# josefmaierfl/matchinglib_poselib

Hardware: AMD Instinct MI355X
Metric: descriptor-pairs/s (8k x 8k ORB BF-Hamming kNN=2 + ratio) (higher is better)
Workload: dtype fp4 (E2M1 MFMA, f32 accumulate: exact); 1 GPU; C2: 8192x8192 ORB-256 BF-Hamming kNN=2 + 0.75 ratio + DMatch rows, 64 image pair(s) per GPU per step; pairs_per_gpu=64, settle_steps=400, solver_polish=1

## Files before the change

include/mlpl_debug.h:

```cpp
#ifndef MLPL_DEBUG_H
#define MLPL_DEBUG_H
#include "mlpl_c.h"

#ifdef __cplusplus
extern "C" {
#endif

int mlpl_debug_arrsac_trace(mlpl_ctx *ctx, int32_t *buf, int cap);

int mlpl_debug_usac_trace(mlpl_ctx *ctx, double *buf, int cap_records);

int mlpl_debug_ransac_draw(mlpl_ctx *ctx, long long out[2]);

long long mlpl_debug_fiber_selftest(int n, int workers, int rounds);

int mlpl_debug_eig9(mlpl_ctx *ctx, const double *G, const double *start, int count, double *out12, double *jacobi10);

int mlpl_debug_dk_stats(mlpl_ctx *ctx, int enable, int stats[16]);

int mlpl_debug_l2_flags(mlpl_ctx *ctx, int flags[4]);

int mlpl_debug_hamming_stamps(mlpl_ctx *ctx, unsigned long long *out, int max_items);

int mlpl_debug_hamming_clock(mlpl_ctx *ctx, unsigned long long *out, int max_items);

int mlpl_debug_hop_trace(mlpl_ctx *ctx, float *us, int *codes, int max_items, long long *ws_grows);

int mlpl_debug_last_kernels(mlpl_ctx *ctx, int out[13]);

int mlpl_debug_last_l2_match(mlpl_ctx *ctx, int out[4]);

int mlpl_debug_l2_fold_counts(mlpl_ctx *ctx, const float *d_q, int nq, size_t q_stride, size_t q_batch_stride, const float *d_t, int nt,
                              size_t t_stride, size_t t_batch_stride, int dim, int ratio_test, float ratio, int batch, int32_t *d_idx, float *d_dist,
                              int32_t *counts);

int mlpl_debug_count_pass(mlpl_ctx *ctx, const double *p1, const double *p2, int n, const double *E, int n_live, int n_bound,
                          const int32_t *ids, int table_len, double thresh2, int point_splits, int32_t *table_inout);

#ifdef __cplusplus
}
#endif
#endif
```

matchinglib_poselib_amd/_lib.py:

```python
from __future__ import annotations

import ctypes as C
import os
import threading

_HERE = os.path.dirname(os.path.abspath(__file__))
_LIB_PATH = os.environ.get("MLPL_LIB_PATH") or os.path.join(_HERE, "lib", "libmlpl_hip.so")

MLPL_OK = 0
MLPL_E_BAD_INPUT = -1
MLPL_E_UNSUPPORTED = -2
MLPL_E_FAILED = -3
MLPL_E_INTERNAL = -103
MLPL_E_FEW_KEYPOINTS = -4
MLPL_E_NO_DEVICE = -100
MLPL_E_HIP = -101
MLPL_E_NOMEM = -102


class MlplError(RuntimeError):
    def __init__(self, code: int, where: str, msg: str = ""):
        self.code = code
        super().__init__(f"{where} failed with code {code}: {msg}")

# ... 76 lines not shown
    "mlpl_usac_essential": (c_int, [c_void_p, c_void_p, c_void_p, c_int, c_void_p, c_void_p, c_void_p, c_void_p]),
    "mlpl_usac_essential_dev": (c_int, [c_void_p, c_void_p, c_void_p, c_int, c_void_p, c_void_p, c_void_p, c_void_p, c_void_p]),
    "mlpl_usac_essential_batch_dev": (c_int, [c_void_p, c_int, c_void_p, c_void_p, c_int, c_void_p, c_void_p, c_void_p, c_void_p, c_void_p, c_void_p,
                                              c_void_p, c_void_p, c_int, c_void_p, c_void_p]),
    "mlpl_usac_last_stats": (c_int, [c_void_p, c_void_p]),
    "mlpl_usac_last_degeneracy": (c_int, [c_void_p, c_void_p, c_void_p, c_void_p, c_int]),
    "mlpl_debug_usac_trace": (c_int, [c_void_p, c_void_p, c_int]),
    "mlpl_ransac_essential": (c_int, [c_void_p, c_void_p, c_void_p, c_int, c_double, c_double, c_int, c_int, c_u32,
                                      c_void_p, c_void_p, C.POINTER(c_int), C.POINTER(c_int)]),
    "mlpl_ransac_essential_dev": (c_int, [c_void_p, c_void_p, c_void_p, c_int, c_double, c_double, c_int, c_int,
                                          c_u32, c_void_p, c_void_p, C.POINTER(c_int), C.POINTER(c_int), c_void_p]),
    "mlpl_solve_5pt": (c_int, [c_void_p, c_void_p, c_void_p, c_int, c_void_p, c_int, c_void_p, c_void_p]),
    "mlpl_score_models": (c_int, [c_void_p, c_void_p, c_void_p, c_int, c_void_p, c_int, c_double, c_void_p,
                                  c_void_p]),
    "mlpl_ransac_last_stats": (c_int, [c_void_p, c_void_p]),
    "mlpl_debug_ransac_draw": (c_int, [c_void_p, c_void_p]),
    "mlpl_debug_fiber_selftest": (C.c_longlong, [c_int, c_int, c_int]),
    "mlpl_debug_eig9": (c_int, [c_void_p, c_void_p, c_void_p, c_int, c_void_p, c_void_p]),
    "mlpl_debug_dk_stats": (c_int, [c_void_p, c_int, c_void_p]),
    "mlpl_debug_hamming_stamps": (c_int, [c_void_p, c_void_p, c_int]),
    "mlpl_debug_hamming_clock": (c_int, [c_void_p, c_void_p, c_int]),
    "mlpl_debug_hop_trace": (c_int, [c_void_p, c_void_p, c_void_p, c_int, c_void_p]),
    "mlpl_debug_last_kernels": (c_int, [c_void_p, c_void_p]),
    "mlpl_debug_count_pass": (c_int, [c_void_p, c_void_p, c_void_p, c_int, c_void_p, c_int, c_int, c_void_p, c_int, c_double, c_int,
                                      c_void_p]),
    "mlpl_pair_pose_dev": (c_int, [c_void_p, c_void_p, c_int, c_void_p, c_int, c_int, c_void_p, c_void_p, c_void_p, c_void_p, c_double,
                                   c_int, c_double, c_int, c_u32, c_double, c_void_p, c_void_p]),
    "mlpl_pair_pose_batch_dev": (c_int, [c_void_p, c_int, c_void_p, c_int, c_void_p, c_int, c_int, c_void_p, c_void_p, c_void_p, c_void_p, c_double,
                                         c_int, c_double, c_int, c_void_p, c_double, c_void_p, c_void_p, c_void_p]),
    "mlpl_pair_pose_f32_dev": (c_int, [c_void_p, c_void_p, c_int, c_void_p, c_int, c_int, c_void_p, c_void_p, c_void_p, c_void_p, c_double,
                                       c_int, c_double, c_int, c_u32, c_double, c_void_p, c_void_p]),
    "mlpl_pair_pose_batch_f32_dev": (c_int, [c_void_p, c_int, c_void_p, c_int, c_void_p, c_int, c_int, c_void_p, c_void_p, c_void_p, c_void_p, c_double,
                                             c_int, c_double, c_int, c_void_p, c_double, c_void_p, c_void_p, c_void_p]),
    "mlpl_pair_pose_batch_usac_f32_dev": (c_int, [c_void_p, c_int, c_void_p, c_int, c_void_p, c_int, c_int, c_void_p, c_void_p, c_void_p, c_void_p, c_void_p, c_int,
                                                  c_void_p, c_double, c_void_p, c_void_p, c_void_p]),
    "mlpl_pair_pose_batch_arrsac_f32_dev": (c_int, [c_void_p, c_int, c_void_p, c_int, c_void_p, c_int, c_int, c_void_p, c_void_p, c_void_p, c_void_p, c_double, c_int,
                                                    c_void_p, c_double, c_void_p, c_void_p, c_void_p]),
    "mlpl_pair_pose_batch_lanes_dev": (c_int, [c_void_p, c_void_p, c_int, c_int, c_void_p, c_int, c_void_p, c_int, c_int, c_void_p, c_void_p, c_void_p, c_void_p,
                                               c_double, c_int, c_double, c_void_p, c_double, c_void_p, c_void_p, c_void_p]),
    "mlpl_pair_pose_batch_usac_dev": (c_int, [c_void_p, c_int, c_void_p, c_int, c_void_p, c_int, c_int, c_void_p, c_void_p, c_void_p, c_void_p, c_void_p, c_int,
                                              c_void_p, c_double, c_void_p, c_void_p, c_void_p]),
    "mlpl_pair_pose_batch_arrsac_dev": (c_int, [c_void_p, c_int, c_void_p, c_int, c_void_p, c_int, c_int, c_void_p, c_void_p, c_void_p, c_void_p, c_double, c_int,
                                                c_void_p, c_double, c_void_p, c_void_p, c_void_p]),
    "mlpl_sorted_match_idx": (c_int, [c_void_p, c_int, c_void_p]),
    "mlpl_pair_batch_last_stats": (c_int, [c_void_p, c_void_p]),
    "mlpl_ransac_essential_batch_dev": (c_int, [c_void_p, c_int, c_void_p, c_void_p, c_int, c_void_p, c_double, c_int, c_double, c_void_p, c_int, c_double,
# ... 112 lines not shown
        return self._lib

    def stream(self) -> int:
        return int(self._lib.mlpl_ctx_stream(self._h) or 0)

    def synchronize(self):
        check(self._lib.mlpl_ctx_synchronize(self._h), "mlpl_ctx_synchronize")

    def set_option(self, name: str, value: int):
        check(self._lib.mlpl_set_option(self._h, name.encode(), int(value)), "mlpl_set_option")

    def get_option(self, name: str) -> int:
        v = C.c_int(0)
        check(self._lib.mlpl_get_option(self._h, name.encode(), C.byref(v)), "mlpl_get_option")
        return v.value

    def last_kernels(self) -> list:
        out = (C.c_int * 13)()
        n = self._lib.mlpl_debug_last_kernels(self._h, out)
        if n < 0:
            raise MlplError(n, "mlpl_debug_last_kernels", last_error())
        return list(out[:n])

    def last_l2_match(self) -> list:
        out = (C.c_int * 4)()
        n = self._lib.mlpl_debug_last_l2_match(self._h, out)
        if n < 0:
            raise MlplError(n, "mlpl_debug_last_l2_match", last_error())
        return list(out[:n])

    def close(self):
        if getattr(self, "_h", None) is not None and self._h:
            self._lib.mlpl_ctx_destroy(self._h)
            self._h = None

    def __del__(self):
        try:
            self.close()
        except Exception:
            pass

    def __enter__(self):
        return self

    def __exit__(self, *exc):
        self.close()
# ... 15 lines not shown
```

matchinglib_poselib_amd/csrc/capi.hip:

```cpp

#include <algorithm>
#include <cfloat>
#include <cstdlib>
#include <cstring>
#include <new>

#include "mlpl_internal.h"

namespace mlpl {

static thread_local char g_err[512] = "";

void set_error(const char *fmt, ...) {
    va_list ap;
    va_start(ap, fmt);
    vsnprintf(g_err, sizeof(g_err), fmt, ap);
    va_end(ap);
}

int ws_get(mlpl_ctx *ctx, WsSlot slot, size_t bytes, void **out) {
    if (bytes < 4096) bytes = 4096;
    if (ctx->ws_bytes[slot] < bytes) {
        MLPL_HIP_TRY(hipDeviceSynchronize());
        if (ctx->ws[slot]) MLPL_HIP_TRY(hipFree(ctx->ws[slot]));
// ... 90 lines not shown
    MLPL_HIP_TRY(hipSetDevice(device_ordinal));
    hipDeviceProp_t prop;
    MLPL_HIP_TRY(hipGetDeviceProperties(&prop, device_ordinal));
    if (std::strncmp(prop.gcnArchName, "gfx950", 6) != 0) {
        set_error("device %d is %s; this library carries gfx950 code objects only", device_ordinal, prop.gcnArchName);
        return MLPL_E_NO_DEVICE;
    }
    mlpl_ctx *ctx = new (std::nothrow) mlpl_ctx();
    if (!ctx) return MLPL_E_NOMEM;
    std::memset(ctx, 0, sizeof(*ctx));
    ctx->device = device_ordinal;
    ctx->num_cus = prop.multiProcessorCount > 0 ? prop.multiProcessorCount : 256;
    ctx->opt_hamming_variant = 3;
    ctx->opt_hamming_qpl = 1;
    ctx->opt_hamming_blocks_per_cu = 32;
    ctx->opt_hamming_mfma_blocks_per_cu = 3;
    ctx->opt_hamming_mfma_qt = 0;
    ctx->opt_hamming_mfma_lds = 1;
    ctx->opt_hamming_mfma_weighted = 1;
    ctx->opt_hamming_mfma_prio = 0;
    ctx->opt_hamming_fused_merge = 1;
    ctx->opt_hamming_expand_fine = 1;
    ctx->opt_hamming_expand_inkernel = 1;
    ctx->opt_hamming_merge_emit = 0;
    ctx->opt_ransac_lazy_sums = 1;
    ctx->opt_ransac_overlap = 1;
    ctx->opt_ransac_f32_filter = 1;
    ctx->opt_ransac_count_mpl = 2;
    ctx->opt_ransac_count_tiles = 2;
    ctx->opt_ransac_count_wpe = 5;
    ctx->opt_ransac_count_threads = 256;
    ctx->opt_ransac_count_defer = 1;
    ctx->opt_pair_batch_feed = 1;
    ctx->opt_solver_polish = 1;
    ctx->opt_solver_wave3 = 1;
    ctx->opt_ransac_device_draw = 1;
    ctx->opt_usac_lo_warm_start = 1;
    ctx->opt_usac_lo5_fused_fit = 1;
    ctx->opt_hub_blocking_sync = 1;
    ctx->opt_eig_inverse_iteration = 1;
    ctx->opt_arrsac_refine_warm_start = 1;
    ctx->opt_usac_sprt_fast = 1;
    ctx->opt_l2_float_mfma = 1;
    ctx->opt_l2_fold_counts = 1;
    ctx->opt_vfc_store_u = 0;
    hipError_t e = hipStreamCreateWithFlags(&ctx->stream, hipStreamNonBlocking);
// ... 40 lines not shown
    if (ctx->stream) (void)hipStreamDestroy(ctx->stream);
    for (int i = 0; i < 2; ++i)
        if (ctx->aux_stream[i]) (void)hipStreamDestroy(ctx->aux_stream[i]);
    for (int i = 0; i < 8; ++i)
        if (ctx->aux_ev[i]) (void)hipEventDestroy(ctx->aux_ev[i]);
    delete ctx;
}

void *mlpl_ctx_stream(mlpl_ctx *ctx) { return ctx ? (void *)ctx->stream : nullptr; }
int mlpl_ctx_device(mlpl_ctx *ctx) { return ctx ? ctx->device : -1; }
int mlpl_ctx_synchronize(mlpl_ctx *ctx) {
    if (!ctx) return MLPL_E_BAD_INPUT;
    MLPL_HIP_TRY(hipStreamSynchronize(ctx->stream));
    return MLPL_OK;
}

static const struct {
    const char *name;
    int mlpl_ctx::*field;
    int lo, hi;
} kRangeOptions[] = {
    {"l2_fold_counts", &mlpl_ctx::opt_l2_fold_counts, 0, 1},
    {"hamming_expand_inkernel", &mlpl_ctx::opt_hamming_expand_inkernel, 0, 1},
    {"vfc_store_u", &mlpl_ctx::opt_vfc_store_u, 0, 1},
};

int mlpl_set_option(mlpl_ctx *ctx, const char *name, int value) {
    if (!ctx || !name) return MLPL_E_BAD_INPUT;
    for (const auto &o : kRangeOptions)
        if (!std::strcmp(name, o.name)) {
            if (value < o.lo || value > o.hi) {
                set_error("mlpl_set_option: unknown option or bad value: %s=%d", name, value);
                return MLPL_E_BAD_INPUT;
            }
            ctx->*(o.field) = value;
            return MLPL_OK;
        }
    if (!std::strcmp(name, "hamming_variant") && value >= 0 && value <= 3) ctx->opt_hamming_variant = value;
    else if (!std::strcmp(name, "hamming_mfma_qt") && (value == 0 || value == 1 || value == 2 || value == 4)) ctx->opt_hamming_mfma_qt = value;
    else if (!std::strcmp(name, "hamming_mfma_blocks_per_cu") && value >= 1 && value <= 64) ctx->opt_hamming_mfma_blocks_per_cu = value;
    else if (!std::strcmp(name, "hamming_mfma_lds") && (value >= 0 && value <= 2)) ctx->opt_hamming_mfma_lds = value;
    else if (!std::strcmp(name, "hamming_expand_fine") && (value == 0 || value == 1)) ctx->opt_hamming_expand_fine = value;
    else if (!std::strcmp(name, "hamming_mfma_prio") && (value == 0 || value == 1 || value == 3)) ctx->opt_hamming_mfma_prio = value;
    else if (!std::strcmp(name, "hamming_mfma_prefetch") && (value == 0 || value == 2 || value == 4 || value == 6)) ctx->opt_hamming_mfma_prefetch = value;
    else if (!std::strcmp(name, "hamming_split_rows") && (value == 0 || value == 4096 || value == 8192)) ctx->opt_hamming_split_rows = value;
    else if (!std::strcmp(name, "hamming_mfma_waves") && (value == 0 || value == 4 || value == 8 || value == 16)) ctx->opt_hamming_mfma_waves = value;
    else if (!std::strcmp(name, "hamming_mfma_weighted") && (value == 0 || value == 1)) ctx->opt_hamming_mfma_weighted = value;
    else if (!std::strcmp(name, "hamming_fused_merge") && (value == 0 || value == 1)) ctx->opt_hamming_fused_merge = value;
    else if (!std::strcmp(name, "hamming_stamps") && (value >= 0 && value <= 2)) ctx->opt_hamming_stamps = value;
    else if (!std::strcmp(name, "hamming_train01") && (value == 0 || value == 1)) ctx->opt_hamming_train01 = value;
    else if (!std::strcmp(name, "hamming_merge_emit") && (value == 0 || value == 1)) ctx->opt_hamming_merge_emit = value;
    else if (!std::strcmp(name, "l2_mfma_waves") && (value == 0 || value == 4 || value == 8)) ctx->opt_l2_mfma_waves = value;
    else if (!std::strcmp(name, "l2_mfma_blocks_per_cu") && value >= 0 && value <= 16) ctx->opt_l2_mfma_blocks_per_cu = value;
    else if (!std::strcmp(name, "hamming_qpl") && (value == 1 || value == 2)) ctx->opt_hamming_qpl = value;
// ... 90 lines not shown
    else if (!std::strcmp(name, "pair_batch_feed")) *value = ctx->opt_pair_batch_feed;
    else if (!std::strcmp(name, "pair_batch_raw_cap")) *value = ctx->opt_pair_batch_raw_cap;
    else if (!std::strcmp(name, "usac_lo_stepwise")) *value = ctx->opt_usac_lo_stepwise;
    else if (!std::strcmp(name, "usac_lo_warm_start")) *value = ctx->opt_usac_lo_warm_start;
    else if (!std::strcmp(name, "usac_first_batch")) *value = ctx->opt_usac_first_batch;
    else if (!std::strcmp(name, "usac_lo5_fused_fit")) *value = ctx->opt_usac_lo5_fused_fit;
    else if (!std::strcmp(name, "usac_sprt_fast")) *value = ctx->opt_usac_sprt_fast;
    else if (!std::strcmp(name, "ransac_host_table")) *value = ctx->opt_ransac_host_table;
    else if (!std::strcmp(name, "ransac_chunk")) *value = ctx->opt_ransac_chunk;
    else {
        set_error("mlpl_get_option: unknown option: %s", name);
        return MLPL_E_BAD_INPUT;
    }
    return MLPL_OK;
}

int mlpl_debug_last_kernels(mlpl_ctx *ctx, int out[13]) {
    if (!ctx || !out) return MLPL_E_BAD_INPUT;
    out[0] = ctx->dbg_count_kernel[0], out[1] = ctx->dbg_count_kernel[1];
    for (int i = 0; i < 11; ++i) out[2 + i] = ctx->dbg_hamming_kernel[i];
    return 13;
}

int mlpl_debug_last_l2_match(mlpl_ctx *ctx, int out[4]) {
    if (!ctx || !out) return MLPL_E_BAD_INPUT;
    for (int i = 0; i < 4; ++i) out[i] = ctx->dbg_l2_match[i];
    return 4;
}

int mlpl_debug_hamming_stamps(mlpl_ctx *ctx, unsigned long long *out, int max_items) {
    if (!ctx || !out) return MLPL_E_BAD_INPUT;
    MLPL_HIP_TRY(hipSetDevice(ctx->device));
    MLPL_HIP_TRY(hipDeviceSynchronize());
    if (max_items < 0) {
        const int n = ctx->dbg_stamp_items < -max_items ? ctx->dbg_stamp_items : -max_items;
        if (n > 0 && ctx->ws[WS_DEBUG])
            MLPL_HIP_TRY(hipMemcpy(out, (char *)ctx->ws[WS_DEBUG] + (size_t)ctx->dbg_stamp_items * 32, (size_t)n * 48 * 8, hipMemcpyDeviceToHost));
        return n;
    }
    const int n = ctx->dbg_stamp_items < max_items ? ctx->dbg_stamp_items : max_items;
    if (n > 0 && ctx->ws[WS_DEBUG]) MLPL_HIP_TRY(hipMemcpy(out, ctx->ws[WS_DEBUG], (size_t)n * 32, hipMemcpyDeviceToHost));
    return n;
}

int mlpl_debug_hop_trace(mlpl_ctx *ctx, float *us, int *codes, int max_items, long long *ws_grows) {
    if (!ctx) return MLPL_E_BAD_INPUT;
// ... 607 lines not shown
```

matchinglib_poselib_amd/csrc/knn_hamming.hip:

```cpp

#include "mlpl_internal.h"

namespace mlpl {

namespace {

constexpr int kQueriesPerBlock = 256;
constexpr int kTileRows = 128;
constexpr int kMergeGroup = 64;
static_assert(kMergeGroup == kCountGroup, "merge kernel and ratio_write_kernel disagree on the count granularity");

constexpr int dist_bits(int nw) {
    int b = 1;
    while ((1 << b) <= nw * 32) ++b;
    return b;
}

__device__ __forceinline__ uint32_t bcnt_acc(uint32_t x, uint32_t acc) {
    uint32_t r;
    asm("v_bcnt_u32_b32 %0, %1, %2" : "=v"(r) : "v"(x), "v"(acc));
    return r;
}

__device__ __forceinline__ uint32_t umed3(uint32_t a, uint32_t b, uint32_t c) {
// ... 432 lines not shown
    const long long target_blocks = (long long)ctx->opt_hamming_blocks_per_cu * ctx->num_cus;
    const int max_split = (nt + kTileRows - 1) / kTileRows;
    long long want = (target_blocks + (long long)qtiles * batch - 1) / ((long long)qtiles * batch);
    int nsplit = (int)std::max<long long>(1, std::min<long long>(want, max_split));
    int rps = (nt + nsplit - 1) / nsplit;
    rps = ((rps + kTileRows - 1) / kTileRows) * kTileRows;
    const int max_rps = ((1 << dshift) - 2) / kTileRows * kTileRows;
    if (rps > max_rps) rps = max_rps;
    nsplit = (nt + rps - 1) / rps;
    if (nsplit > 65535) {
        set_error("knn_hamming: train set too large (nt=%d)", nt);
        return MLPL_E_BAD_INPUT;
    }

    void *part = nullptr;
    int rc = ws_get(ctx, WS_PARTIAL, (size_t)batch * nsplit * nq * sizeof(uint2), &part);
    if (rc) return rc;

    dim3 grid(qtiles, nsplit, batch);
    {
        int *rec = ctx->dbg_hamming_kernel;
        rec[0] = variant, rec[1] = (variant == 1 && nw <= 16) ? qpl : 1, rec[2] = 0, rec[3] = 0, rec[4] = 0;
        rec[5] = 0, rec[6] = 0, rec[7] = 0, rec[8] = nsplit, rec[9] = 0, rec[10] = 0;
    }
    prof_mark(ctx, MLPL_PROF_KNN_HAMMING, 0, s);
    switch (nw) {
        case 1: launch_partial<1>(variant, qpl, grid, s, qw, qbw, tw, tbw, nq, nt, rps, nsplit, (uint2 *)part); break;
        case 2: launch_partial<2>(variant, qpl, grid, s, qw, qbw, tw, tbw, nq, nt, rps, nsplit, (uint2 *)part); break;
        case 4: launch_partial<4>(variant, qpl, grid, s, qw, qbw, tw, tbw, nq, nt, rps, nsplit, (uint2 *)part); break;
        case 8: launch_partial<8>(variant, qpl, grid, s, qw, qbw, tw, tbw, nq, nt, rps, nsplit, (uint2 *)part); break;
        case 16: launch_partial<16>(variant, qpl, grid, s, qw, qbw, tw, tbw, nq, nt, rps, nsplit, (uint2 *)part); break;
        case 32: launch_partial<32>(variant, qpl, grid, s, qw, qbw, tw, tbw, nq, nt, rps, nsplit, (uint2 *)part); break;
        case 64: launch_partial<64>(variant, qpl, grid, s, qw, qbw, tw, tbw, nq, nt, rps, nsplit, (uint2 *)part); break;
        default: set_error("knn_hamming: unsupported descriptor width %d bytes", nbytes); return MLPL_E_BAD_INPUT;
    }
    prof_mark(ctx, MLPL_PROF_KNN_HAMMING, 1, s);
    launch_merge(s, (const uint2 *)part, nq, nsplit, rps, dshift, k, ratio, batch, d_idx, d_dist, d_group_counts);
    MLPL_HIP_TRY(hipGetLastError());
    return MLPL_OK;
}

}
```

matchinglib_poselib_amd/csrc/knn_hamming_mfma.hip:

```cpp

#include <algorithm>
#include <cmath>
#include <type_traits>
#include <vector>

#include "mlpl_internal.h"


namespace mlpl {

namespace {

typedef int v8i __attribute__((ext_vector_type(8)));
typedef float v16f __attribute__((ext_vector_type(16)));
typedef uint32_t u32x4 __attribute__((ext_vector_type(4)));
typedef uint32_t u32x2 __attribute__((ext_vector_type(2)));

constexpr float kEps = 1.0f / 16384.0f;
constexpr int kMaxRowsPerSplit = 8192;

__device__ __forceinline__ float fmax_raw(float a, float b) {
    float r;
    asm("v_max_f32 %0, %1, %2" : "=v"(r) : "v"(a), "v"(b));
    return r;
// ... 102 lines not shown
}

#ifndef MLPL_MFMA_SCALED
#define MLPL_MFMA_SCALED 0
#endif
__device__ __forceinline__ v16f mfma_fp4(uint4 a, uint4 b, v16f c) {
    const v8i av = {(int)a.x, (int)a.y, (int)a.z, (int)a.w, 0, 0, 0, 0};
    const v8i bv = {(int)b.x, (int)b.y, (int)b.z, (int)b.w, 0, 0, 0, 0};
#if MLPL_MFMA_SCALED
    return __builtin_amdgcn_mfma_scale_f32_32x32x64_f8f6f4(av, bv, c, 4, 4, 0, 0x7F7F7F7F, 0, 0x7F7F7F7F);
#else
    return __builtin_amdgcn_mfma_scale_f32_32x32x64_f8f6f4(av, bv, c, 4, 4, 0, 0, 0, 0);
#endif
}

__device__ __forceinline__ void top2_update4(float &m1, float &m2, float a0, float a1, float a2, float a3) {
    const float s0 = __builtin_amdgcn_fmed3f(m1, a0, a1);
    const float t0 = __builtin_fmaxf(__builtin_fmaxf(m1, a0), a1);
    const float s1 = __builtin_amdgcn_fmed3f(t0, a2, a3);
    m1 = __builtin_fmaxf(__builtin_fmaxf(t0, a2), a3);
    m2 = __builtin_fmaxf(__builtin_fmaxf(m2, s0), s1);
}

__device__ __forceinline__ int acc_local_row(int reg, int h) { return (reg & 3) + 8 * (reg >> 2) + 4 * h; }
__device__ __forceinline__ v16f row_weights(int h) {
    v16f c;
#pragma unroll
    for (int reg = 0; reg < 16; ++reg) c[reg] = -(float)acc_local_row(reg, h) * kEps;
    return c;
}
__device__ __forceinline__ v16f row_weights_ragged(int h, int tile_row0, int nt) {
    v16f c;
#pragma unroll
    for (int reg = 0; reg < 16; ++reg) {
        const int lr = acc_local_row(reg, h);
        c[reg] = (tile_row0 + lr < nt) ? -(float)lr * kEps : -INFINITY;
    }
    return c;
}

struct DistRule {
    int nbits;
    int train01;
    int qpop;
    __device__ __forceinline__ int operator()(int ip) const { return train01 ? qpop - ip : (nbits - ip) >> 1; }
};
__device__ __forceinline__ uint32_t decode_key(float v, float frame, int dshift, DistRule dist) {
    const float ip = rintf(v);
    const int d = dist((int)ip);
    const int lrow = (int)(frame - (v - ip) * 16384.0f);
    return ((uint32_t)d << dshift) | (uint32_t)lrow;
}
__device__ __forceinline__ uint2 top2_across_halves(const uint32_t (&k)[2]) {
    const uint32_t o0 = __shfl_xor(k[0], 32), o1 = __shfl_xor(k[1], 32);
    uint32_t k0 = k[0], k1 = k[1];
    k1 = umed3(k0, k1, o0);
    k0 = min(k0, o0);
    k1 = umed3(k0, k1, o1);
    k0 = min(k0, o1);
    return make_uint2(k0, k1);
}

__device__ __forceinline__ int xcd_block_item() {
    const int per_xcd = (int)(gridDim.x >> 3);
    return (int)(blockIdx.x & 7) * per_xcd + (int)(blockIdx.x >> 3);
}

__device__ __forceinline__ void clock_start(bool on, unsigned long long &st_c, unsigned long long &st_r) {
    if (on) {
        st_c = __builtin_amdgcn_s_memtime();
        st_r = __builtin_amdgcn_s_memrealtime();
    }
}
__device__ __forceinline__ void clock_stamp(unsigned long long *o, unsigned long long st_c, unsigned long long st_r, int tiles, int qt) {
    o[0] = __builtin_amdgcn_s_memtime() - st_c;
    o[1] = __builtin_amdgcn_s_memrealtime() - st_r;
    const unsigned hw = __builtin_amdgcn_s_getreg(4 | (0 << 6) | (31 << 11)), xcc = __builtin_amdgcn_s_getreg(20 | (0 << 6) | (3 << 11));
    o[2] = (unsigned long long)tiles * qt | ((unsigned long long)(hw & 0xFFFFFu) << 32) | ((unsigned long long)(xcc & 15u) << 56);
    o[3] = st_r;
}

__device__ __forceinline__ void ring_read_tile(u32x4 (&r)[4], uint32_t addr) {
    asm volatile(
// ... 90 lines not shown
    for (int t = 0; t < QT; ++t) {
        uint32_t k[2];
        const float mm[2] = {m1[t], m2[t]};
#pragma unroll
        for (int j = 0; j < 2; ++j)
            k[j] = mm[j] == -INFINITY ? 0xFFFFFFFFu : decode_key(mm[j], frame, dshift, DistRule{64 * KS, 0, 0});
        const uint2 kk = top2_across_halves(k);
        const int q = (qt0 + t) * 32 + (l & 31);
        if (h == 0 && q < nq) part[((size_t)b * nsplit + split) * nq + q] = kk;
    }
    if (stamps && l == 0) clock_stamp(stamps + (size_t)item * 4, st_c, st_r, ntiles, QT);
}

struct HammingFuse {
    int32_t *idx, *dist, *group_counts;
    int *tickets;
    int k;
    float ratio;
    int train01;
    unsigned long long *clk;
    unsigned long long launch_no;
};

template <int QT, int PRIO, int NW = 4, int PD = 2, bool XP = false, bool ST = false>
__global__ __launch_bounds__(64 * NW, 4) void knn_hamming_mfma_lds_kernel(
    const uint32_t *__restrict__ qw, size_t q_batch_words, const void *__restrict__ tsrc, size_t t_batch, int nq, int nt,
    int rows_per_split, int nsplit, int dshift, int qblocks, int n_items, uint2 *__restrict__ part,
    unsigned long long *__restrict__ stamps, const int32_t *__restrict__ split_tile0, HammingFuse fuse) {
    constexpr int KS = 4, NB = XP ? 2 : PD == 2 ? 4 : 8, NR = 4;
    static_assert(PD == 2 || PD == 4 || PD == 6, "prefetch distance");
    static_assert(!XP || (NW == 8 && PD == 2), "the in-kernel expansion exists for eight waves and a prefetch distance of 2");
    __shared__ __attribute__((aligned(16))) uint4 ring[NB][KS * 64];
    __shared__ __attribute__((aligned(16))) uint32_t raw_ring[XP ? NR * 256 : 1];
    const int l = threadIdx.x & 63;
    const int w = __builtin_amdgcn_readfirstlane((int)(threadIdx.x >> 6));
    unsigned long long st_c = 0, st_r = 0;
    clock_start(stamps || fuse.clk, st_c, st_r);
    const int item = xcd_block_item();
    if (item >= n_items) return;
    const int qb = item % qblocks;
    const int split = (item / qblocks) % nsplit;
    const int b = item / (qblocks * nsplit);
    const int qt0 = (qb * NW + w) * QT;
    const int h = l >> 5;

    uint4 bq[QT][KS];
    v16f cinit;
#pragma unroll
    for (int reg = 0; reg < 16; ++reg) cinit[reg] = -(float)acc_local_row(reg, h) * kEps;

    int row0 = split * rows_per_split;
    int row1 = min(nt, row0 + rows_per_split);
    if (split_tile0) {
        row0 = 32 * split_tile0[(size_t)b * (nsplit + 1) + split];
// ... 31 lines not shown
        xp_raw = raw_lds + (uint32_t)w * 4u + (lx >> 1) * 32u;
        xp_plane = frag_lds + (uint32_t)(w & 3) * 1024u + (uint32_t)(w >> 2) * 512u + lx * 8u;
        xp_sh = lx & 1u;
        xp_voff = PD * 1024u + (uint32_t)w * 256u + lx * 4u;
        asm volatile("" : "+v"(xp_frag), "+v"(xp_raw), "+v"(xp_plane), "+v"(xp_sh), "+v"(xp_voff));
    }
    auto raw_addr = [&](int t_rel) { return xp_raw + (uint32_t)((t_rel + NR - 1) & (NR - 1)) * 1024u; };
    auto plane_addr = [&](int t_rel) { return xp_plane + (uint32_t)(t_rel & 1) * (KS * 1024u); };
    auto expand_pair = [&](uint32_t x) {
        const uint32_t y = x >> xp_sh;
        return u32x2{expand_plane0(y, 0x22222222u), expand_plane2(y, 0x22222222u)};
    };
    auto tile_math = [&](const u32x4 (&r)[KS], const v16f &c0) {
        uint4 a[KS];
#pragma unroll
        for (int s = 0; s < KS; ++s) a[s] = make_uint4(r[s].x, r[s].y, r[s].z, r[s].w);
#pragma unroll
        for (int t = 0; t < QT; ++t) {
            v16f acc = mfma_fp4(a[0], bq[t][0], c0);
#pragma unroll
            for (int s = 1; s < KS; ++s) acc = mfma_fp4(a[s], bq[t][s], acc);
            m1[t] += 32.0f * kEps;
            m2[t] += 32.0f * kEps;
#pragma unroll
            for (int reg = 0; reg < 16; reg += 4) {
                if constexpr (PRIO == 3) {
                    const float g = __builtin_fmaxf(__builtin_fmaxf(__builtin_fmaxf(acc[reg], acc[reg + 1]), acc[reg + 2]), acc[reg + 3]);
                    if (__builtin_amdgcn_ballot_w64(g > m2[t]) == 0) continue;
                }
                top2_update4(m1[t], m2[t], acc[reg], acc[reg + 1], acc[reg + 2], acc[reg + 3]);
            }
        }
    };
    auto tile_body = [&](int it, const v16f &c0) {
        u32x4 r[KS];
        const uint32_t addr = (XP ? xp_frag : ring_lds) + (uint32_t)(it & (NB - 1)) * (KS * 1024u);
        if constexpr (XP) {
            uint32_t x;
            const uint32_t ra = raw_addr(it + 1), wa = plane_addr(it + 1);
            asm volatile(
                "ds_read_b32 %4, %6\n\tds_read_b128 %0, %5\n\tds_read_b128 %1, %5 offset:1024\n\tds_read_b128 %2, %5 offset:2048\n\t"
                "ds_read_b128 %3, %5 offset:3072"
                : "=&v"(r[0]), "=&v"(r[1]), "=&v"(r[2]), "=&v"(r[3]), "=&v"(x)
                : "v"(addr), "v"(ra)
                : "memory");
            asm volatile("s_waitcnt lgkmcnt(4)" : "+v"(x));
// ... 137 lines not shown
    }

    int le = l_end, qt0e = qt0;
    asm volatile("" : "+v"(le), "+s"(qt0e));
    const int he = le >> 5;
    const float frame = (float)(32 * (ntiles - 1));
    int pass_acc = 0;
#pragma unroll
    for (int t = 0; t < QT; ++t) {
        int qpop = 0;
        if (fuse.train01) {
            const int row = (qt0e + t) * 32 + (le & 31);
            uint4 v = make_uint4(0u, 0u, 0u, 0u);
            if (row < nq) v = *reinterpret_cast<const uint4 *>(qw + (size_t)b * q_batch_words + (size_t)row * (2 * KS) + (size_t)he * KS);
            const int pc = __popc(v.x) + __popc(v.y) + __popc(v.z) + __popc(v.w);
            qpop = pc + __shfl_xor(pc, 32);
        }
        uint32_t k[2];
        const float mm[2] = {m1[t], m2[t]};
#pragma unroll
        for (int j = 0; j < 2; ++j)
            k[j] = mm[j] == -INFINITY ? 0xFFFFFFFFu : decode_key(mm[j], frame, dshift, DistRule{64 * KS, fuse.train01, qpop});
        const uint2 kk = top2_across_halves(k);
        const uint32_t k0 = kk.x, k1 = kk.y;
        const int q = (qt0e + t) * 32 + (le & 31);
        if (fuse.idx && nsplit == 1) {
            const uint32_t lmask = (1u << dshift) - 1u;
            bool pass = false;
            if (he == 0 && q < nq) {
                const size_t o = ((size_t)b * nq + q) * fuse.k;
                const int d0 = k0 == 0xFFFFFFFFu ? -1 : (int)(k0 >> dshift);
                fuse.idx[o] = k0 == 0xFFFFFFFFu ? -1 : (int)(row0 + (k0 & lmask));
                fuse.dist[o] = d0;
                if (fuse.k == 2) {
                    const int d1 = k1 == 0xFFFFFFFFu ? -1 : (int)(k1 >> dshift);
                    fuse.idx[o + 1] = k1 == 0xFFFFFFFFu ? -1 : (int)(row0 + (k1 & lmask));
                    fuse.dist[o + 1] = d1;
                    pass = (float)d0 < __fmul_rn(fuse.ratio, (float)d1);
                } else {
                    pass = true;
                }
            }
            const int c = __popcll(__ballot(pass));
            pass_acc = (t & 1) ? pass_acc + c : c;
            if (fuse.group_counts && (t & 1) && le == 0 && (qt0e + t - 1) * 32 < nq) fuse.group_counts[(size_t)b * ((nq + 63) >> 6) + ((qt0e + t) >> 1)] = pass_acc;
        } else if (he == 0 && q < nq) {
            if (fuse.idx)
                __hip_atomic_store(reinterpret_cast<unsigned long long *>(&part[((size_t)b * nsplit + split) * nq + q]),
// ... 212 lines not shown
template <class F>
void dispatch_ks(int ks, F &&f) {
    switch (ks) {
        case 1: f(int_c<1>{}); break;
        case 2: f(int_c<2>{}); break;
        case 4: f(int_c<4>{}); break;
        default: f(int_c<8>{}); break;
    }
}

struct RingLaunch {
    dim3 grid;
    hipStream_t s;
    const uint32_t *qw;
    size_t q_batch_words;
    const void *tsrc;
    size_t t_batch;
    int nq, nt, rps, nsplit, dshift, qblocks, n_items;
    uint2 *part;
    unsigned long long *stamps;
    const int32_t *split_tab;
    HammingFuse fuse;
};
template <int QT, int PRIO, int NW = 4, int PD = 2, bool XP = false, bool ST = false>
void launch_ring(const RingLaunch &a) {
    hipLaunchKernelGGL((knn_hamming_mfma_lds_kernel<QT, PRIO, NW, PD, XP, ST>), a.grid, dim3(64 * NW), 0, a.s, a.qw, a.q_batch_words, a.tsrc,
                       a.t_batch, a.nq, a.nt, a.rps, a.nsplit, a.dshift, a.qblocks, a.n_items, a.part, a.stamps, a.split_tab, a.fuse);
}

bool age_aware_split_table(unsigned grid_x, long long items, int num_cus, int qblocks, int nsplit, int batch, int t_tiles, int max_rps,
                           std::vector<int32_t> &tab) {
    const int per_xcd = (int)(grid_x >> 3);
    tab.assign((size_t)batch * (nsplit + 1), -1);
    for (long long bid = 0; bid < items; ++bid) {
        const long long item = (bid & 7) * per_xcd + (bid >> 3);
        if (item >= items) continue;
        const int sp = (int)((item / qblocks) % nsplit), bb = (int)(item / ((long long)qblocks * nsplit));
        const int r = (int)(bid / num_cus);
        int32_t &slot = tab[(size_t)bb * (nsplit + 1) + sp];
        if (slot < 0) slot = r;
        else if (slot != r) return false;
    }
    static const double kRate[4] = {1.0 / 1700, 1.0 / 2100, 1.0 / 3200, 1.0 / 5300};
    for (int bb = 0; bb < batch; ++bb) {
        int32_t *h = tab.data() + (size_t)bb * (nsplit + 1);
        double wsum = 0;
        for (int sp = 0; sp < nsplit; ++sp) wsum += kRate[h[sp]];
        int acc_tiles = 0;
        double acc_w = 0;
// ... 60 lines not shown
        const long long teams = (long long)qblocks * nspan * batch;
        const long long want_mem = ((long long)bpc * ctx->num_cus + teams - 1) / teams;
        nmem = (int)std::max<long long>(1, std::min<long long>(want_mem, (span_tiles + chunk_tiles - 1) / chunk_tiles));
        nsplit = nspan * nmem;
        rps = span_tiles * 32;
        sps = nmem;
        if (nsplit > 65535) {
            set_error("knn_hamming: train set too large (nt=%d)", nt);
            return MLPL_E_BAD_INPUT;
        }
    }
    const long long items = (lds_ring ? (long long)qblocks : (long long)qgroups) * nsplit * batch;
    if (items > (1LL << 30)) {
        set_error("knn_hamming: problem too large for one launch (nq=%d nt=%d batch=%d)", nq, nt, batch);
        return MLPL_E_BAD_INPUT;
    }

    const int pd = (nwv == 8 && (ctx->opt_hamming_mfma_prefetch == 4 || ctx->opt_hamming_mfma_prefetch == 6)) ? ctx->opt_hamming_mfma_prefetch : 2;
    const int prio = (nwv == 16 || pd != 2) ? 0 : ctx->opt_hamming_mfma_prio == 1 ? 1 : (ctx->opt_hamming_mfma_prio == 3 && nwv == 8) ? 3 : 0;
    const int train01 = (lds_ring && !dyn && ctx->opt_hamming_train01) ? 1 : 0;
    const bool inkernel = ctx->opt_hamming_expand_inkernel && lds_ring && !dyn && nwv == 8 && pd == 2 && prio == 0 && nw == 8 && !train01 &&
                          ((uintptr_t)tw & 3u) == 0;

    void *qf = nullptr, *tf = nullptr, *part = nullptr;
    int rc;
    const size_t q_u4 = (size_t)q_tiles_padded * ks * 64, t_u4 = (size_t)t_tiles * ks * 64;
    if ((rc = ws_get(ctx, WS_FRAG_Q, (size_t)batch * q_u4 * 16, &qf))) return rc;
    if (!inkernel && (rc = ws_get(ctx, WS_FRAG_T, ((size_t)batch * t_u4 + (size_t)ks * 64) * 16, &tf))) return rc;
    if ((rc = ws_get(ctx, WS_PARTIAL, (size_t)batch * nsplit * nq * sizeof(uint2), &part))) return rc;
    int *counters = nullptr;
    const int counters_per_batch = dyn ? qblocks * nspan : 0;
    if (dyn) {
        void *cp = nullptr;
        if ((rc = ws_get(ctx, WS_COUNTERS, (size_t)batch * counters_per_batch * sizeof(int), &cp))) return rc;
        counters = (int *)cp;
    }
    const bool expand_q = !(lds_ring && !dyn);
    const ExpandArgs ta{tw, t_batch_words, nt, t_tiles, (uint4 *)tf};
    const ExpandArgs qa = expand_q ? ExpandArgs{qw, q_batch_words, nq, q_tiles_padded, (uint4 *)qf} : ta;
    const dim3 egrid((unsigned)(((expand_q ? std::max(q_tiles_padded, t_tiles) : t_tiles) * 64 + 255) / 256), batch, expand_q ? 2 : 1);
    const bool expand_fine = !inkernel && !expand_q && ks == 4 && nw == 8 && !counters && (long long)t_tiles * batch <= 4LL * ctx->num_cus && ctx->opt_hamming_expand_fine;
    if (inkernel) {
    } else if (expand_fine) {
        hipLaunchKernelGGL(hamming_expand_fine_kernel, dim3((unsigned)t_tiles, batch), dim3(256), 0, s, ta, train01);
    } else {
        dispatch_ks(ks, [&](auto KS) {
// ... 47 lines not shown
            }
            fuse.tickets = (int *)tp;
        }
        *fused_out = 1;
    }
    {
        int *rec = ctx->dbg_hamming_kernel;
        rec[0] = dyn ? 5 : lds_ring ? 4 : 3, rec[1] = (dyn || !lds_ring) ? (ks <= 4 && qt == 4 ? 4 : qt >= 2 ? 2 : 1) : qt;
        rec[2] = (lds_ring && !dyn) ? prio : 0, rec[3] = lds_ring && !dyn ? nwv : 4, rec[4] = lds_ring && !dyn ? pd : 0;
        rec[5] = *fused_out, rec[6] = split_tab != nullptr, rec[7] = expand_fine, rec[8] = nsplit, rec[9] = ks, rec[10] = inkernel;
    }
    prof_mark(ctx, MLPL_PROF_KNN_HAMMING, 0, s);
    if (dyn) {
        auto launch_dyn = [&](auto QT) {
            hipLaunchKernelGGL((knn_hamming_mfma_dyn_kernel<decltype(QT)::value>), grid, dim3(256), 0, s, (const uint4 *)qf, q_u4, (const uint4 *)tf, t_u4, nq,
                               nt, span_tiles, nspan, nmem, chunk_tiles, dshift, qblocks, (int)items, (uint2 *)part, counters, stamps);
        };
        if (qt == 4) launch_dyn(int_c<4>{});
        else if (qt == 2) launch_dyn(int_c<2>{});
        else launch_dyn(int_c<1>{});
    } else if (lds_ring) {
        const RingLaunch ra{grid, s, qw, q_batch_words, inkernel ? (const void *)tw : (const void *)tf, inkernel ? t_batch_words : t_u4, nq, nt, rps, nsplit,
                            dshift, qblocks, (int)items, (uint2 *)part, stamps, split_tab, fuse};
        if (inkernel && stamps) launch_ring<4, 0, 8, 2, true, true>(ra);
        else if (inkernel) launch_ring<4, 0, 8, 2, true>(ra);
        else if (nwv == 16) launch_ring<4, 0, 16>(ra);
        else if (nwv == 8 && pd == 4) launch_ring<4, 0, 8, 4>(ra);
        else if (nwv == 8 && pd == 6) launch_ring<4, 0, 8, 6>(ra);
        else if (nwv == 8 && prio == 3) launch_ring<4, 3, 8>(ra);
        else if (nwv == 8 && prio == 1) launch_ring<4, 1, 8>(ra);
        else if (nwv == 8) launch_ring<4, 0, 8>(ra);
        else if (qt == 4) prio == 1 ? launch_ring<4, 1>(ra) : launch_ring<4, 0>(ra);
        else if (qt == 2) prio == 1 ? launch_ring<2, 1>(ra) : launch_ring<2, 0>(ra);
        else prio == 1 ? launch_ring<1, 1>(ra) : launch_ring<1, 0>(ra);
    } else {
        dispatch_ks(ks, [&](auto KS) {
            auto launch_mfma = [&](auto QT) {
                hipLaunchKernelGGL((knn_hamming_mfma_kernel<decltype(KS)::value, decltype(QT)::value>), grid, dim3(256), 0, s, (const uint4 *)qf, q_u4,
                                   (const uint4 *)tf, t_u4, nq, nt, rps, nsplit, dshift, qgroups, (int)items, (uint2 *)part, stamps);
            };
            if constexpr (decltype(KS)::value <= 4) {
                if (qt == 4) return launch_mfma(int_c<4>{});
            }
            if (qt >= 2) launch_mfma(int_c<2>{});
            else launch_mfma(int_c<1>{});
        });
    }
    prof_mark(ctx, MLPL_PROF_KNN_HAMMING, 1, s);
// ... 11 lines not shown
```

matchinglib_poselib_amd/csrc/mlpl_internal.h:

```cpp
#pragma once

#include <hip/hip_runtime.h>

#include <cstdarg>
#include <cstddef>
#include <cstdint>
#include <cstdio>

#include "mlpl_c.h"
#include "mlpl_debug.h"

namespace mlpl {

void set_error(const char *fmt, ...);

#define MLPL_HIP_TRY(expr)                                                                                  \
    do {                                                                                                    \
        hipError_t e__ = (expr);                                                                            \
        if (e__ != hipSuccess) {                                                                            \
            ::mlpl::set_error("%s:%d: %s -> %s", __FILE__, __LINE__, #expr, hipGetErrorString(e__));        \
            return MLPL_E_HIP;                                                                              \
        }                                                                                                   \
    } while (0)

// ... 85 lines not shown
    int opt_hamming_mfma_blocks_per_cu;
    int opt_hamming_mfma_qt;
    int opt_hamming_mfma_lds;
    int opt_hamming_mfma_waves;
    int opt_hamming_split_rows;
    int opt_hamming_mfma_prefetch;
    int opt_hamming_mfma_prio;
    int opt_hamming_mfma_weighted;
    long long split_tab_key;
    void *split_tab_ptr;
    int opt_hamming_fused_merge;
    void *hamming_tickets_ptr;
    size_t hamming_tickets_bytes;
    int opt_hamming_expand_fine;
    int opt_hamming_stamps;
    long long hamming_clock_launches;
    int opt_hamming_merge_emit;
    void *hamming_scan_ptr;
    size_t hamming_scan_bytes;
    uint32_t hamming_scan_gen;
    int opt_hamming_train01;
    int opt_vfc_store_u;
    int opt_hamming_expand_inkernel;
    void *subpix_sep_mask_ptr;
    int dbg_stamp_items;
    int dbg_count_kernel[2];
    int dbg_hamming_kernel[11];
    int opt_ransac_chunk;
    int opt_ransac_event_cap;
    int opt_ransac_count_mpl;
    int opt_ransac_count_threads;
    int opt_ransac_count_wpe;
    int opt_ransac_count_tiles;
    int opt_ransac_count_defer;
    int opt_ransac_f32_filter;
    int opt_ransac_overlap;
    int opt_ransac_dev_split;
    int opt_ransac_lazy_sums;
    int opt_solver_polish;
    int opt_solver_wave3;
    int opt_ransac_host_table;
    int opt_rand_cache_max;
    void *rand_cache;
    int32_t *ransac_T_host;
    int ransac_T_n;
    double ransac_T_conf;
// ... 183 lines not shown
```

Baseline: 11980 billion descriptor-pairs/s.

## Track top-2 over 4-row blocks in MFMA Hamming loop and rescan best block

```diff
diff --git a/include/mlpl_debug.h b/include/mlpl_debug.h
--- a/include/mlpl_debug.h
+++ b/include/mlpl_debug.h
@@ -28,6 +28,8 @@
 
 int mlpl_debug_last_kernels(mlpl_ctx *ctx, int out[13]);
 
+int mlpl_debug_last_hamming_top2(mlpl_ctx *ctx);
+
 int mlpl_debug_last_l2_match(mlpl_ctx *ctx, int out[4]);
 
 int mlpl_debug_l2_fold_counts(mlpl_ctx *ctx, const float *d_q, int nq, size_t q_stride, size_t q_batch_stride, const float *d_t, int nt,
diff --git a/matchinglib_poselib_amd/_lib.py b/matchinglib_poselib_amd/_lib.py
--- a/matchinglib_poselib_amd/_lib.py
+++ b/matchinglib_poselib_amd/_lib.py
@@ -122,6 +122,7 @@
     "mlpl_debug_hamming_clock": (c_int, [c_void_p, c_void_p, c_int]),
     "mlpl_debug_hop_trace": (c_int, [c_void_p, c_void_p, c_void_p, c_int, c_void_p]),
     "mlpl_debug_last_kernels": (c_int, [c_void_p, c_void_p]),
+    "mlpl_debug_last_hamming_top2": (c_int, [c_void_p]),
     "mlpl_debug_count_pass": (c_int, [c_void_p, c_void_p, c_void_p, c_int, c_void_p, c_int, c_int, c_void_p, c_int, c_double, c_int,
                                       c_void_p]),
     "mlpl_pair_pose_dev": (c_int, [c_void_p, c_void_p, c_int, c_void_p, c_int, c_int, c_void_p, c_void_p, c_void_p, c_void_p, c_double,
@@ -280,6 +281,12 @@
             raise MlplError(n, "mlpl_debug_last_kernels", last_error())
         return list(out[:n])
 
+    def last_hamming_top2(self) -> int:
+        n = self._lib.mlpl_debug_last_hamming_top2(self._h)
+        if n < 0:
+            raise MlplError(n, "mlpl_debug_last_hamming_top2", last_error())
+        return n
+
     def last_l2_match(self) -> list:
         out = (C.c_int * 4)()
         n = self._lib.mlpl_debug_last_l2_match(self._h, out)
diff --git a/matchinglib_poselib_amd/csrc/capi.hip b/matchinglib_poselib_amd/csrc/capi.hip
--- a/matchinglib_poselib_amd/csrc/capi.hip
+++ b/matchinglib_poselib_amd/csrc/capi.hip
@@ -136,6 +136,7 @@
     ctx->opt_hamming_fused_merge = 1;
     ctx->opt_hamming_expand_fine = 1;
     ctx->opt_hamming_expand_inkernel = 1;
+    ctx->opt_hamming_block_top2 = 4;
     ctx->opt_hamming_merge_emit = 0;
     ctx->opt_ransac_lazy_sums = 1;
     ctx->opt_ransac_overlap = 1;
@@ -222,6 +223,7 @@
 } kRangeOptions[] = {
     {"l2_fold_counts", &mlpl_ctx::opt_l2_fold_counts, 0, 1},
     {"hamming_expand_inkernel", &mlpl_ctx::opt_hamming_expand_inkernel, 0, 1},
+    {"hamming_block_top2", &mlpl_ctx::opt_hamming_block_top2, 0, 4},
     {"vfc_store_u", &mlpl_ctx::opt_vfc_store_u, 0, 1},
 };
 
@@ -229,7 +231,8 @@
     if (!ctx || !name) return MLPL_E_BAD_INPUT;
     for (const auto &o : kRangeOptions)
         if (!std::strcmp(name, o.name)) {
-            if (value < o.lo || value > o.hi) {
+            const bool bad_block = o.field == &mlpl_ctx::opt_hamming_block_top2 && value != 0 && value != 4;
+            if (value < o.lo || value > o.hi || bad_block) {
                 set_error("mlpl_set_option: unknown option or bad value: %s=%d", name, value);
                 return MLPL_E_BAD_INPUT;
             }
@@ -366,6 +369,8 @@
     return 13;
 }
 
+int mlpl_debug_last_hamming_top2(mlpl_ctx *ctx) { return ctx ? ctx->dbg_hamming_top2 : MLPL_E_BAD_INPUT; }
+
 int mlpl_debug_last_l2_match(mlpl_ctx *ctx, int out[4]) {
     if (!ctx || !out) return MLPL_E_BAD_INPUT;
     for (int i = 0; i < 4; ++i) out[i] = ctx->dbg_l2_match[i];
diff --git a/matchinglib_poselib_amd/csrc/knn_hamming.hip b/matchinglib_poselib_amd/csrc/knn_hamming.hip
--- a/matchinglib_poselib_amd/csrc/knn_hamming.hip
+++ b/matchinglib_poselib_amd/csrc/knn_hamming.hip
@@ -478,6 +478,7 @@
         int *rec = ctx->dbg_hamming_kernel;
         rec[0] = variant, rec[1] = (variant == 1 && nw <= 16) ? qpl : 1, rec[2] = 0, rec[3] = 0, rec[4] = 0;
         rec[5] = 0, rec[6] = 0, rec[7] = 0, rec[8] = nsplit, rec[9] = 0, rec[10] = 0;
+        ctx->dbg_hamming_top2 = 0;
     }
     prof_mark(ctx, MLPL_PROF_KNN_HAMMING, 0, s);
     switch (nw) {
diff --git a/matchinglib_poselib_amd/csrc/knn_hamming_mfma.hip b/matchinglib_poselib_amd/csrc/knn_hamming_mfma.hip
--- a/matchinglib_poselib_amd/csrc/knn_hamming_mfma.hip
+++ b/matchinglib_poselib_amd/csrc/knn_hamming_mfma.hip
@@ -148,6 +148,17 @@
     m2 = __builtin_fmaxf(__builtin_fmaxf(m2, s0), s1);
 }
 
+__device__ __forceinline__ void top2_update_blocks4(float &m1, float &m2, const v16f &acc) {
+    auto max4 = [&](int j) { return __builtin_fmaxf(__builtin_fmaxf(__builtin_fmaxf(acc[4 * j], acc[4 * j + 1]), acc[4 * j + 2]), acc[4 * j + 3]); };
+    const float g0 = max4(0), g1 = max4(1);
+    const float s0 = __builtin_amdgcn_fmed3f(m1, g0, g1);
+    const float t0 = __builtin_fmaxf(__builtin_fmaxf(m1, g0), g1);
+    const float g2 = max4(2), g3 = max4(3);
+    const float s1 = __builtin_amdgcn_fmed3f(t0, g2, g3);
+    m1 = __builtin_fmaxf(__builtin_fmaxf(t0, g2), g3);
+    m2 = __builtin_fmaxf(__builtin_fmaxf(m2, s0), s1);
+}
+
 __device__ __forceinline__ int acc_local_row(int reg, int h) { return (reg & 3) + 8 * (reg >> 2) + 4 * h; }
 __device__ __forceinline__ v16f row_weights(int h) {
     v16f c;
@@ -185,6 +196,26 @@
     k1 = umed3(k0, k1, o1);
     k0 = min(k0, o1);
     return make_uint2(k0, k1);
+}
+
+struct __attribute__((packed, aligned(4))) RawRow {
+    uint32_t w[8];
+};
+__device__ __forceinline__ uint32_t block_rescan(uint32_t k0, const uint32_t (&q8)[8], const char *rbase, int rows, int dshift, int he) {
+    const uint32_t lmask = (1u << dshift) - 1u;
+    const int best = (int)(k0 & lmask);
+    uint32_t res = 0xFFFFFFFFu;
+#pragma unroll
+    for (int i = 0; i < 2; ++i) {
+        const int r = (best & ~3) + 2 * he + i;
+        const RawRow t = *reinterpret_cast<const RawRow *>(rbase + (size_t)min(r, rows - 1) * 32);
+        int d = 0;
+#pragma unroll
+        for (int j = 0; j < 8; ++j) d += __popc(t.w[j] ^ q8[j]);
+        const uint32_t key = ((uint32_t)d << dshift) | (uint32_t)r;
+        res = (r != best && r < rows && k0 != 0xFFFFFFFFu) ? min(res, key) : res;
+    }
+    return min(res, (uint32_t)__shfl_xor(res, 32));
 }
 
 __device__ __forceinline__ int xcd_block_item() {
@@ -321,7 +352,7 @@
     unsigned long long launch_no;
 };
 
-template <int QT, int PRIO, int NW = 4, int PD = 2, bool XP = false, bool ST = false>
+template <int QT, int PRIO, int NW = 4, int PD = 2, bool XP = false, bool ST = false, int BT = 0>
 __global__ __launch_bounds__(64 * NW, 4) void knn_hamming_mfma_lds_kernel(
     const uint32_t *__restrict__ qw, size_t q_batch_words, const void *__restrict__ tsrc, size_t t_batch, int nq, int nt,
     int rows_per_split, int nsplit, int dshift, int qblocks, int n_items, uint2 *__restrict__ part,
@@ -329,6 +360,7 @@
     constexpr int KS = 4, NB = XP ? 2 : PD == 2 ? 4 : 8, NR = 4;
     static_assert(PD == 2 || PD == 4 || PD == 6, "prefetch distance");
     static_assert(!XP || (NW == 8 && PD == 2), "the in-kernel expansion exists for eight waves and a prefetch distance of 2");
+    static_assert(BT == 0 || (XP && PRIO == 0 && BT == 4), "the block update needs the raw train rows of the in-kernel expansion");
     __shared__ __attribute__((aligned(16))) uint4 ring[NB][KS * 64];
     __shared__ __attribute__((aligned(16))) uint32_t raw_ring[XP ? NR * 256 : 1];
     const int l = threadIdx.x & 63;
@@ -406,6 +438,11 @@
             for (int s = 1; s < KS; ++s) acc = mfma_fp4(a[s], bq[t][s], acc);
             m1[t] += 32.0f * kEps;
             m2[t] += 32.0f * kEps;
+            if constexpr (BT == 4) {
+                top2_update_blocks4(m1[t], m2[t], acc);
+                asm volatile("" : "+v"(m1[t]), "+v"(m2[t]), "+v"(a[0].x));
+                continue;
+            }
 #pragma unroll
             for (int reg = 0; reg < 16; reg += 4) {
                 if constexpr (PRIO == 3) {
@@ -589,8 +626,20 @@
         for (int j = 0; j < 2; ++j)
             k[j] = mm[j] == -INFINITY ? 0xFFFFFFFFu : decode_key(mm[j], frame, dshift, DistRule{64 * KS, fuse.train01, qpop});
         const uint2 kk = top2_across_halves(k);
-        const uint32_t k0 = kk.x, k1 = kk.y;
         const int q = (qt0e + t) * 32 + (le & 31);
+        const uint32_t k0 = kk.x;
+        uint32_t k1 = kk.y;
+        if constexpr (BT != 0) {
+            if (fuse.k != 1) {
+                uint32_t q8[8] = {0u, 0u, 0u, 0u, 0u, 0u, 0u, 0u};
+                if (q < nq) {
+                    const uint4 *qp = reinterpret_cast<const uint4 *>(qw + (size_t)b * q_batch_words + (size_t)q * (2 * KS));
+                    const uint4 v0 = qp[0], v1 = qp[1];
+                    q8[0] = v0.x, q8[1] = v0.y, q8[2] = v0.z, q8[3] = v0.w, q8[4] = v1.x, q8[5] = v1.y, q8[6] = v1.z, q8[7] = v1.w;
+                }
+                k1 = min(k1, block_rescan(k0, q8, rbase, nt - row0, dshift, he));
+            }
+        }
         if (fuse.idx && nsplit == 1) {
             const uint32_t lmask = (1u << dshift) - 1u;
             bool pass = false;
@@ -849,9 +898,9 @@
     const int32_t *split_tab;
     HammingFuse fuse;
 };
-template <int QT, int PRIO, int NW = 4, int PD = 2, bool XP = false, bool ST = false>
+template <int QT, int PRIO, int NW = 4, int PD = 2, bool XP = false, bool ST = false, int BT = 0>
 void launch_ring(const RingLaunch &a) {
-    hipLaunchKernelGGL((knn_hamming_mfma_lds_kernel<QT, PRIO, NW, PD, XP, ST>), a.grid, dim3(64 * NW), 0, a.s, a.qw, a.q_batch_words, a.tsrc,
+    hipLaunchKernelGGL((knn_hamming_mfma_lds_kernel<QT, PRIO, NW, PD, XP, ST, BT>), a.grid, dim3(64 * NW), 0, a.s, a.qw, a.q_batch_words, a.tsrc,
                        a.t_batch, a.nq, a.nt, a.rps, a.nsplit, a.dshift, a.qblocks, a.n_items, a.part, a.stamps, a.split_tab, a.fuse);
 }
 
@@ -958,6 +1007,9 @@
     const bool inkernel = ctx->opt_hamming_expand_inkernel && lds_ring && !dyn && nwv == 8 && pd == 2 && prio == 0 && nw == 8 && !train01 &&
                           ((uintptr_t)tw & 3u) == 0;
 
+    const int block_top2 = inkernel ? ctx->opt_hamming_block_top2 : 0;
+    ctx->dbg_hamming_top2 = block_top2;
+
     void *qf = nullptr, *tf = nullptr, *part = nullptr;
     int rc;
     const size_t q_u4 = (size_t)q_tiles_padded * ks * 64, t_u4 = (size_t)t_tiles * ks * 64;
@@ -1051,8 +1103,10 @@
     } else if (lds_ring) {
         const RingLaunch ra{grid, s, qw, q_batch_words, inkernel ? (const void *)tw : (const void *)tf, inkernel ? t_batch_words : t_u4, nq, nt, rps, nsplit,
                             dshift, qblocks, (int)items, (uint2 *)part, stamps, split_tab, fuse};
-        if (inkernel && stamps) launch_ring<4, 0, 8, 2, true, true>(ra);
-        else if (inkernel) launch_ring<4, 0, 8, 2, true>(ra);
+        if (inkernel && stamps)
+            block_top2 == 4 ? launch_ring<4, 0, 8, 2, true, true, 4>(ra) : launch_ring<4, 0, 8, 2, true, true>(ra);
+        else if (inkernel)
+            block_top2 == 4 ? launch_ring<4, 0, 8, 2, true, false, 4>(ra) : launch_ring<4, 0, 8, 2, true>(ra);
         else if (nwv == 16) launch_ring<4, 0, 16>(ra);
         else if (nwv == 8 && pd == 4) launch_ring<4, 0, 8, 4>(ra);
         else if (nwv == 8 && pd == 6) launch_ring<4, 0, 8, 6>(ra);
diff --git a/matchinglib_poselib_amd/csrc/mlpl_internal.h b/matchinglib_poselib_amd/csrc/mlpl_internal.h
--- a/matchinglib_poselib_amd/csrc/mlpl_internal.h
+++ b/matchinglib_poselib_amd/csrc/mlpl_internal.h
@@ -131,6 +131,8 @@
     int opt_hamming_train01;
     int opt_vfc_store_u;
     int opt_hamming_expand_inkernel;
+    int opt_hamming_block_top2;
+    int dbg_hamming_top2;
     void *subpix_sep_mask_ptr;
     int dbg_stamp_items;
     int dbg_count_kernel[2];
```

Measured after the change: 12630 billion descriptor-pairs/s (median of 6 runs). +5.5%, better.
